# yizuo417/RollingDepth

Hardware: AMD Instinct MI355X
Metric: depth frames/sec at 768px snip_len=3, 1-step denoise; 1/2/4/8 MI355X (higher is better)
Workload: dtype f16; 1 GPU; fast preset: 100-frame 768x768 video, dilations [1, 25] (cap_dilation=True), snippet_len 3, 1-step DDIM, aligner 2000 it, refine 0; SD2-shaped UNet+VAE random-init; preset=fast, frames=100, res=768, parallelism=snippet-dp1

## Files before the change

### include/rdmi.h

```cpp
#ifndef RDMI_H
#define RDMI_H

#include <stddef.h>

#ifdef __cplusplus
extern "C" {
#endif

#define RDMI_OK 0
#define RDMI_E_ARG 1001
#define RDMI_E_ALIGN 1002
#define RDMI_E_UNSUPPORTED 1003

#define RDMI_F16 0
#define RDMI_F32 1
#define RDMI_U8 2
#define RDMI_F32_X3 3
#define RDMI_F32_X6 4

#define RDMI_RESIZE_NEAREST 0
#define RDMI_RESIZE_BILINEAR 1
#define RDMI_RESIZE_BICUBIC 2

#define RDMI_EPI_NONE 0
#define RDMI_EPI_GEGLU 1
#define RDMI_EPI_SILU 2

const char* rdmi_last_error(void);
int rdmi_version(void);

typedef struct rdmi_gemm_args {
  const void* A; long lda; long strideA;
  const void* W; long ldw; long strideW;
  void* C; long ldc; long strideC; int c_f32;
  const float* bias;
  const void* residual; long ldr; long strideR;
  const float* rowbias; int rows_per_group; long rowbias_ld;
  float alpha;
  int M, N, K, batch;
  int epilogue;
  float* gn_part; long gn_ld;
  int dtype;
} rdmi_gemm_args;
int rdmi_gemm(const rdmi_gemm_args* args, void* stream);

typedef struct rdmi_conv_args {
  const void* x; const void* w; void* y;
  const float* bias; const void* residual; const float* rowbias;
  int B, H, W, Cin, Cout, kh, kw, stride, pad_top, pad_left, upsample, Ho, Wo, Kp;
  long y_ld; long res_ld; float alpha; long rowbias_ld;
  float* gn_part; long gn_ld;
  const float* in_mean_rstd; const float* in_gamma; const float* in_beta; int in_groups, in_silu;
  int dtype;
  const void* w_up2;
  const float* in_affine;
} rdmi_conv_args;
int rdmi_conv2d(const rdmi_conv_args* args, void* stream);
int rdmi_conv2d_in_gn_supported(const rdmi_conv_args* args);

long rdmi_groupnorm_workspace(int B, int G);
int rdmi_groupnorm_stats(const void* x, int dtype, int B, long HW, int C, int G, float eps,
                         float* mean_rstd, float* workspace, void* stream);
int rdmi_groupnorm_stats_partials(const float* part, long part_ld, int B, long HW, int C, int G, float eps,
                                  float* mean_rstd, void* stream);
int rdmi_groupnorm_affine(const float* mean_rstd, const float* gamma, const float* beta, int B, int C, int G,
                          float* out, void* stream);
int rdmi_groupnorm_apply(const void* x, void* y, int dtype, int B, long HW, int C, int G,
                         const float* mean_rstd, const float* gamma, const float* beta, int silu,
                         void* stream);

long rdmi_conv3x3_to1_gn_workspace(int B, int H, int W);
int rdmi_conv3x3_to1_gn(const void* x, int dtype, int B, int H, int W, int C, int G, const float* mean_rstd,
                        const float* gamma, const float* beta, int silu, const float* w, float bias,
                        void* y, int y_dtype, float* workspace, void* stream);

int rdmi_layernorm(const void* x, void* y, int dtype, long M, int C, const float* gamma, const float* beta,
                   float eps, void* stream);

int rdmi_attention_fwd(const void* q, const void* k, const void* v, void* o, int B, int H, int Sq,
                       int Sk, int D, long q_ld, long k_ld, long v_ld, long o_ld, long q_bs,
                       long k_bs, long v_bs, long o_bs, float scale, int dtype, void* stream);

int rdmi_attention_smallkv(const void* q, const void* k, const void* v, void* o, int B, int H,
                           int Sq, int L, int D, long q_ld, long o_ld, long q_bs, long o_bs,
                           long kv_bs, float scale, int dtype, void* stream);

int rdmi_cross_attn_pair(const void* x, void* y, long M, int C, int H, const float* ln_gamma,
                         const float* ln_beta, float eps, const float* w, const float* u, const float* c,
                         void* stream);

int rdmi_softmax_rows(const float* s, void* p, long rows, long cols, long p_ld, float scale, int p_dtype,
                      void* stream);

int rdmi_nchw_to_nhwc(const void* x, int x_f32, void* y, int y_dtype, int B, int C, int H, int W, int Cpad,
                      float scale, long x_bstride, long x_cstride, void* stream);
int rdmi_nhwc_to_nchw_f32(const void* x, int dtype, long ld, float* y, int B, int C, int H, int W,
                          float scale, float shift, void* stream);
int rdmi_concat_channels(const void* a, int Ca, const void* b, int Cb, void* y, long P, int dtype, void* stream);
int rdmi_resize_nearest(const void* x, int B, int H, int W, int C, void* y, int Ho, int Wo, int dtype,
                        void* stream);
int rdmi_transpose(const void* src, void* dst, int batch, long rows, long cols, long src_ld,
                   long dst_ld, int dtype, void* stream);
int rdmi_gather_unet_input(const void* rgb, long rgb_frame_ld, const void* depth,
                           long depth_frame_ld, int depth_bcast, const int* frame_idx, int count,
                           long HW, void* out, int dtype, void* stream);
int rdmi_ddim_combine(const void* x, long ld_x, const void* e, long ld_e, void* y, long ld_y,
                      long P, int C, int Cpad, float ca, float cb, float out_scale, long e_period,
                      int dtype, void* stream);
int rdmi_snippet_average(const void* src, int n, int w, int stride, int N, long P, int C, int ld,
                         void* out, int dtype, void* stream);
int rdmi_colorize(const void* depth, int dtype, long n, const void* minmax, const unsigned char* lut, int lut_n,
                  unsigned char* rgb, int* index, void* stream);
int rdmi_snippet_accumulate(const void* src, int dtype, int k0, int nloc, int w, int stride, int N, long P, int C,
                            int ld, double* sum, void* stream);
int rdmi_snippet_finish(const double* sum, int n, int w, int stride, int N, long P, int C, int ld, void* out,
                        int dtype, void* stream);
int rdmi_snippet_average_strided(const void* src, int n, int w, int stride, int start_step, int N, long P, int C,
                                 int ld, void* out, int dtype, void* stream);
int rdmi_snippet_accumulate_strided(const void* src, int dtype, int k0, int nloc, int w, int stride, int start_step,
                                    int N, long P, int C, int ld, double* sum, void* stream);
int rdmi_snippet_finish_strided(const double* sum, int n, int w, int stride, int start_step, int N, long P, int C,
                                int ld, void* out, int dtype, void* stream);
int rdmi_minmax(const void* x, int x_f32, long n, float* minmax, float* workspace, void* stream);
int rdmi_renormalize_f32(float* x, long n, const float* minmax, void* stream);

typedef struct rdmi_aligner_args {
  int n_dil;
  const float* x[8];
  float* s[8]; float* t[8];
  int n[8]; int stride[8];
  int w[8];
  int seq_len; long P;
  float lr, beta1, beta2, eps, lmda2, lmda3, depth_w, loss_scale;
  int iters;
  float* history;
  float* workspace;
  int start_step[8];
} rdmi_aligner_args;
long rdmi_aligner_workspace(const rdmi_aligner_args* a);
int rdmi_aligner_optimize(const rdmi_aligner_args* a, void* stream);
int rdmi_aligner_prepare(const void* x, int x_f32, int n, int w, int H, int W, int border,
                         int factor, const float* shift, float* out, void* stream);
int rdmi_aligner_merge(int n_dil, const void* const* xf, int x_f32, const float* const* s,
                       const float* const* t, const int* n, const int* stride, const int* w, int seq_len,
                       long HW, const float* shift, float* out, void* stream);
int rdmi_aligner_merge_strided(int n_dil, const void* const* xf, int x_f32, const float* const* s,
                               const float* const* t, const int* n, const int* stride, const int* start_step,
                               const int* w, int seq_len, long HW, const float* shift, float* out, void* stream);

int rdmi_aligner_merge_partial_window(int n_dil, const void* const* xf, int x_f32, const float* const* s,
                                      const float* const* t, const int* n, const int* stride, const int* k0,
                                      const int* nloc, const int* w, int f0, int nf, long HW, const float* shift,
                                      double* sum_out, void* stream);
int rdmi_aligner_merge_finish_pieces(int n_dil, const int* n, const int* stride, const int* w, int f0, int nf, long HW,
                                     int npieces, const int* piece_f0, const int* piece_nf, const double* recv,
                                     float* out, void* stream);
int rdmi_aligner_merge_partial_window_strided(int n_dil, const void* const* xf, int x_f32, const float* const* s,
                                              const float* const* t, const int* n, const int* stride,
                                              const int* start_step, const int* k0, const int* nloc, const int* w,
                                              int seq_len, int f0, int nf, long HW, const float* shift,
                                              double* sum_out, void* stream);
int rdmi_aligner_merge_finish_pieces_strided(int n_dil, const int* n, const int* stride, const int* start_step,
                                             const int* w, int seq_len, int f0, int nf, long HW, int npieces,
                                             const int* piece_f0, const int* piece_nf, const double* recv,
                                             float* out, void* stream);

int rdmi_attention_d512(const void* q, const void* k, const void* vt, void* o, int B, int Sq, int Sk, int Skp,
                        long q_ld, long k_ld, long vt_ld, long o_ld, long q_bs, long k_bs, long vt_bs, long o_bs,
                        float scale, int* flags, void* stream);

size_t rdmi_resize_workspace(int N, int C, int H, int W, int Ho, int Wo);
// ... 8 lines not shown
```

### rollingdepth_amd/_native.py

```python
from __future__ import annotations

import ctypes as C
import os

_LIB_PATH = os.environ.get("RDMI_LIB") or os.path.join(os.path.dirname(os.path.abspath(__file__)), "_lib", "librdmi.so")

vp = C.c_void_p
i32 = C.c_int
i64 = C.c_long
f32 = C.c_float


class GemmArgs(C.Structure):
    _fields_ = [
        ("A", vp), ("lda", i64), ("strideA", i64),
        ("W", vp), ("ldw", i64), ("strideW", i64),
        ("C", vp), ("ldc", i64), ("strideC", i64), ("c_f32", i32),
        ("bias", vp),
        ("residual", vp), ("ldr", i64), ("strideR", i64),
        ("rowbias", vp), ("rows_per_group", i32), ("rowbias_ld", i64),
        ("alpha", f32),
        ("M", i32), ("N", i32), ("K", i32), ("batch", i32),
        ("epilogue", i32),
        ("gn_part", vp), ("gn_ld", i64),
        ("dtype", i32),
    ]


class ConvArgs(C.Structure):
    _fields_ = [
        ("x", vp), ("w", vp), ("y", vp),
        ("bias", vp), ("residual", vp), ("rowbias", vp),
        ("B", i32), ("H", i32), ("W", i32), ("Cin", i32), ("Cout", i32), ("kh", i32), ("kw", i32),
        ("stride", i32), ("pad_top", i32), ("pad_left", i32), ("upsample", i32), ("Ho", i32), ("Wo", i32),
        ("Kp", i32),
        ("y_ld", i64), ("res_ld", i64), ("alpha", f32), ("rowbias_ld", i64),
        ("gn_part", vp), ("gn_ld", i64),
        ("in_mean_rstd", vp), ("in_gamma", vp), ("in_beta", vp), ("in_groups", i32), ("in_silu", i32),
        ("dtype", i32),
        ("w_up2", vp),
        ("in_affine", vp),
    ]


class AlignerArgs(C.Structure):
    _fields_ = [
        ("n_dil", i32),
        ("x", vp * 8), ("s", vp * 8), ("t", vp * 8),
        ("n", i32 * 8), ("stride", i32 * 8),
        ("w", i32 * 8), ("seq_len", i32), ("P", i64),
        ("lr", f32), ("beta1", f32), ("beta2", f32), ("eps", f32), ("lmda2", f32), ("lmda3", f32),
        ("depth_w", f32), ("loss_scale", f32),
        ("iters", i32),
        ("history", vp), ("workspace", vp),
        ("start_step", i32 * 8),
    ]


_SIGS = {
    "rdmi_last_error": (C.c_char_p, []),
    "rdmi_version": (i32, []),
    "rdmi_gemm": (i32, [C.POINTER(GemmArgs), vp]),
    "rdmi_conv2d": (i32, [C.POINTER(ConvArgs), vp]),
    "rdmi_conv2d_in_gn_supported": (i32, [C.POINTER(ConvArgs)]),
    "rdmi_groupnorm_workspace": (i64, [i32, i32]),
    "rdmi_groupnorm_stats": (i32, [vp, i32, i32, i64, i32, i32, f32, vp, vp, vp]),
    "rdmi_groupnorm_stats_partials": (i32, [vp, i64, i32, i64, i32, i32, f32, vp, vp]),
    "rdmi_groupnorm_apply": (i32, [vp, vp, i32, i32, i64, i32, i32, vp, vp, vp, i32, vp]),
    "rdmi_conv3x3_to1_gn_workspace": (i64, [i32, i32, i32]),
    "rdmi_conv3x3_to1_gn": (i32, [vp, i32, i32, i32, i32, i32, i32, vp, vp, vp, i32, vp, f32, vp, i32, vp, vp]),
    "rdmi_layernorm": (i32, [vp, vp, i32, i64, i32, vp, vp, f32, vp]),
    "rdmi_attention_fwd": (i32, [vp, vp, vp, vp, i32, i32, i32, i32, i32, i64, i64, i64, i64, i64, i64, i64, i64,
                                 f32, i32, vp]),
    "rdmi_attention_smallkv": (i32, [vp, vp, vp, vp, i32, i32, i32, i32, i32, i64, i64, i64, i64, i64, f32, i32, vp]),
    "rdmi_cross_attn_pair": (i32, [vp, vp, i64, i32, i32, vp, vp, f32, vp, vp, vp, vp]),
    "rdmi_softmax_rows": (i32, [vp, vp, i64, i64, i64, f32, i32, vp]),
    "rdmi_nchw_to_nhwc": (i32, [vp, i32, vp, i32, i32, i32, i32, i32, i32, f32, i64, i64, vp]),
    "rdmi_nhwc_to_nchw_f32": (i32, [vp, i32, i64, vp, i32, i32, i32, i32, f32, f32, vp]),
    "rdmi_concat_channels": (i32, [vp, i32, vp, i32, vp, i64, i32, vp]),
    "rdmi_resize_nearest": (i32, [vp, i32, i32, i32, i32, vp, i32, i32, i32, vp]),
    "rdmi_transpose": (i32, [vp, vp, i32, i64, i64, i64, i64, i32, vp]),
    "rdmi_gather_unet_input": (i32, [vp, i64, vp, i64, i32, vp, i32, i64, vp, i32, vp]),
    "rdmi_ddim_combine": (i32, [vp, i64, vp, i64, vp, i64, i64, i32, i32, f32, f32, f32, i64, i32, vp]),
    "rdmi_snippet_average": (i32, [vp, i32, i32, i32, i32, i64, i32, i32, vp, i32, vp]),
    "rdmi_snippet_accumulate": (i32, [vp, i32, i32, i32, i32, i32, i32, i64, i32, i32, vp, vp]),
    "rdmi_snippet_finish": (i32, [vp, i32, i32, i32, i32, i64, i32, i32, vp, i32, vp]),
    "rdmi_snippet_average_strided": (i32, [vp, i32, i32, i32, i32, i32, i64, i32, i32, vp, i32, vp]),
    "rdmi_snippet_accumulate_strided": (i32, [vp, i32, i32, i32, i32, i32, i32, i32, i64, i32, i32, vp, vp]),
    "rdmi_snippet_finish_strided": (i32, [vp, i32, i32, i32, i32, i32, i64, i32, i32, vp, i32, vp]),
    "rdmi_colorize": (i32, [vp, i32, i64, vp, vp, i32, vp, vp, vp]),
    "rdmi_resize_workspace": (C.c_size_t, [i32, i32, i32, i32, i32, i32]),
    "rdmi_attention_d512": (i32, [vp, vp, vp, vp, i32, i32, i32, i32] + [i64] * 8 + [C.c_float, vp, vp]),
    "rdmi_resize": (i32, [vp, i32, i64, i64, i64, i64, i32, i32, i32, i32, i32, i32, i32, i32, vp, vp, vp]),
    "rdmi_minmax": (i32, [vp, i32, i64, vp, vp, vp]),
    "rdmi_renormalize_f32": (i32, [vp, i64, vp, vp]),
    "rdmi_aligner_workspace": (i64, [C.POINTER(AlignerArgs)]),
    "rdmi_aligner_optimize": (i32, [C.POINTER(AlignerArgs), vp]),
    "rdmi_aligner_prepare": (i32, [vp, i32, i32, i32, i32, i32, i32, i32, vp, vp, vp]),
    "rdmi_aligner_merge": (i32, [i32, C.POINTER(vp), i32, C.POINTER(vp), C.POINTER(vp), C.POINTER(i32),
                                 C.POINTER(i32), C.POINTER(i32), i32, i64, vp, vp, vp]),
    "rdmi_aligner_merge_strided": (i32, [i32, C.POINTER(vp), i32, C.POINTER(vp), C.POINTER(vp), C.POINTER(i32),
                                         C.POINTER(i32), C.POINTER(i32), C.POINTER(i32), i32, i64, vp, vp, vp]),
    "rdmi_groupnorm_affine": (i32, [vp, vp, vp, i32, i32, i32, vp, vp]),
    "rdmi_aligner_merge_partial_window": (i32, [i32, C.POINTER(vp), i32, C.POINTER(vp), C.POINTER(vp),
                                                C.POINTER(i32), C.POINTER(i32), C.POINTER(i32), C.POINTER(i32),
                                                C.POINTER(i32), i32, i32, i64, vp, vp, vp]),
    "rdmi_aligner_merge_finish_pieces": (i32, [i32, C.POINTER(i32), C.POINTER(i32), C.POINTER(i32), i32, i32, i64,
                                               i32, C.POINTER(i32), C.POINTER(i32), vp, vp, vp]),
    "rdmi_aligner_merge_partial_window_strided": (i32, [i32, C.POINTER(vp), i32, C.POINTER(vp), C.POINTER(vp),
                                                        C.POINTER(i32), C.POINTER(i32), C.POINTER(i32),
                                                        C.POINTER(i32), C.POINTER(i32), C.POINTER(i32), i32, i32, i32,
                                                        i64, vp, vp, vp]),
    "rdmi_aligner_merge_finish_pieces_strided": (i32, [i32, C.POINTER(i32), C.POINTER(i32), C.POINTER(i32),
                                                       C.POINTER(i32), i32, i32, i32, i64, i32, C.POINTER(i32),
                                                       C.POINTER(i32), vp, vp, vp]),
}

RDMI_F16, RDMI_F32, RDMI_U8, RDMI_F32_X3, RDMI_F32_X6 = 0, 1, 2, 3, 4
RDMI_RESIZE_NEAREST, RDMI_RESIZE_BILINEAR, RDMI_RESIZE_BICUBIC = 0, 1, 2

EXPORTED = tuple(_SIGS)


def _load():
    if not os.path.exists(_LIB_PATH):
        raise ImportError(
            f"librdmi.so not found at {_LIB_PATH}: build it with `python -m rollingdepth_amd._build` "
            "(the HIP path has no fallback)")
    lib = C.CDLL(_LIB_PATH)
    for name, (res, args) in _SIGS.items():
        fn = getattr(lib, name)
        fn.restype = res
        fn.argtypes = args
    return lib


lib = _load()


class RdmiError(RuntimeError):
    pass


def check(rc: int, what: str = ""):
    if rc != 0:
        msg = lib.rdmi_last_error().decode(errors="replace")
        raise RdmiError(f"{what or 'librdmi'} failed (code {rc}): {msg}")
```

### rollingdepth_amd/csrc/attention.hip

```cpp
#include <stdlib.h>

#include <type_traits>

#include "common.h"

namespace {

struct AttnP {
  const f16* q; const f16* k; const f16* v; f16* o;
  int H, Sq, Sk;
  long q_ld, k_ld, v_ld, o_ld, q_bs, k_bs, v_bs, o_bs;
  float sl2;
  unsigned long long* stamps;
  int sprio;
};

__device__ __forceinline__ unsigned long long attn_stamp() {
  unsigned long long t;
  __builtin_amdgcn_sched_barrier(0);
  asm volatile("s_memtime %0\n\ts_waitcnt lgkmcnt(0)" : "=s"(t) :: "memory");
  __builtin_amdgcn_sched_barrier(0);
  return t;
}

// ... 776 lines not shown
    if constexpr (HC > 0) wave_sum_n<1>(qr, b2); else qr[0] = wave_sum(q);
    const float rstd = rsqrtf(qr[0] / C + eps);
    float n[NV][8], o[NV][8];
#pragma unroll
    for (int i = 0; i < NV; ++i)
#pragma unroll
      for (int e = 0; e < 8; ++e) {
        n[i][e] = lane + 64 * i < CV ? (float)(f16)(((float)v[i][e] - mean) * rstd * gr[i][e] + br[i][e]) : 0.f;
        o[i][e] = 0.f;
      }
    if constexpr (HC > 0) {
      float d[HC];
#pragma unroll
      for (int h = 0; h < HC; ++h) {
        d[h] = 0.f;
#pragma unroll
        for (int i = 0; i < NV; ++i) {
          const int cv = lane + 64 * i;
          if (cv < CV) {
            const f32x4 w0 = *(const f32x4*)(ws + h * C + cv * 8), w1 = *(const f32x4*)(ws + h * C + cv * 8 + 4);
#pragma unroll
            for (int e = 0; e < 4; ++e) d[h] = fmaf(n[i][e], w0[e], fmaf(n[i][4 + e], w1[e], d[h]));
          }
        }
      }
      wave_sum_n<HC>(d, b2);
#pragma unroll
      for (int h = 0; h < HC; ++h) {
        const float ph = 1.0f / (1.0f + __expf(-d[h]));
#pragma unroll
        for (int i = 0; i < NV; ++i) {
          const int cv = lane + 64 * i;
          if (cv < CV) {
            const f32x4 u0 = *(const f32x4*)(us + h * C + cv * 8), u1 = *(const f32x4*)(us + h * C + cv * 8 + 4);
#pragma unroll
            for (int e = 0; e < 4; ++e) {
              o[i][e] = fmaf(ph, u0[e], o[i][e]);
              o[i][4 + e] = fmaf(ph, u1[e], o[i][4 + e]);
            }
          }
        }
      }
    }
    for (int h = 0; h < (HC > 0 ? 0 : H); ++h) {
      float d = 0.f;
#pragma unroll
      for (int i = 0; i < NV; ++i) {
        const int cv = lane + 64 * i;
        if (cv < CV) {
          const f32x4 w0 = *(const f32x4*)(ws + h * C + cv * 8), w1 = *(const f32x4*)(ws + h * C + cv * 8 + 4);
#pragma unroll
          for (int e = 0; e < 4; ++e) d = fmaf(n[i][e], w0[e], fmaf(n[i][4 + e], w1[e], d));
        }
      }
      d = wave_sum(d);
      const float ph = 1.0f / (1.0f + __expf(-d));
#pragma unroll
      for (int i = 0; i < NV; ++i) {
        const int cv = lane + 64 * i;
        if (cv < CV) {
          const f32x4 u0 = *(const f32x4*)(us + h * C + cv * 8), u1 = *(const f32x4*)(us + h * C + cv * 8 + 4);
#pragma unroll
          for (int e = 0; e < 4; ++e) {
            o[i][e] = fmaf(ph, u0[e], o[i][e]);
            o[i][4 + e] = fmaf(ph, u1[e], o[i][4 + e]);
          }
        }
      }
    }
    f16* yr = y + row * C;
#pragma unroll
    for (int i = 0; i < NV; ++i) {
      const int cv = lane + 64 * i;
      if (cv < CV) {
        f16x8 r;
#pragma unroll
        for (int e = 0; e < 8; ++e) r[e] = (f16)((float)v[i][e] + (cr[i][e] + o[i][e]));
        *(f16x8*)(yr + cv * 8) = r;
      }
    }
  }
}

}

extern "C" int rdmi_attention_fwd(const void* q, const void* k, const void* v, void* o, int B, int H, int Sq, int Sk,
                                  int D, long q_ld, long k_ld, long v_ld, long o_ld, long q_bs, long k_bs, long v_bs,
                                  long o_bs, float scale, int dtype, void* stream) {
  RDMI_REQUIRE(q && k && v && o, RDMI_E_ARG, "attention_fwd: null pointer");
  RDMI_REQUIRE(D == 64, RDMI_E_UNSUPPORTED, "attention_fwd: head_dim %d unsupported (64 only)", D);
  RDMI_REQUIRE(B > 0 && H > 0 && Sq > 0 && Sk > 0, RDMI_E_ARG, "attention_fwd: bad sizes");
  if (dtype == RDMI_F32 || dtype == RDMI_F32_X3 || dtype == RDMI_F32_X6)
    return rdmi::attention_fwd_f32(q, k, v, o, B, H, Sq, Sk, q_ld, k_ld, v_ld, o_ld, q_bs, k_bs, v_bs, o_bs, scale,
                                   dtype == RDMI_F32_X3 ? 2 : dtype == RDMI_F32_X6 ? 3 : 1, stream);
  RDMI_REQUIRE(q_ld % 8 == 0 && k_ld % 8 == 0 && v_ld % 8 == 0 && o_ld % 4 == 0 && (((uintptr_t)q | (uintptr_t)k | (uintptr_t)v) & 15) == 0,
               RDMI_E_ALIGN, "attention_fwd: strides/pointers must be 16-byte aligned");
  AttnP p{(const f16*)q, (const f16*)k, (const f16*)v, (f16*)o, H, Sq, Sk, q_ld, k_ld, v_ld, o_ld, q_bs, k_bs, v_bs, o_bs,
          scale * 1.4426950408889634f, nullptr};
  const char* sp = getenv("RDMI_ATTN_SPRIO");
  p.sprio = sp && sp[0] == '1';
  dim3 g(rdmi::div_up(Sq, QB), H, B);
  static const bool f32sum = [] { const char* e = getenv("RDMI_ATTN_F32SUM"); return e && e[0] == '1'; }();
  const char* pe = getenv("RDMI_ATTN_PIPE");
  if (pe && pe[0] == '1' && !f32sum) {
    hipLaunchKernelGGL((attn_fwd_d64_pipe<0, true>), dim3(rdmi::div_up(Sq, pp::QB), H, B), dim3(64 * pp::NW), 0,
                       (hipStream_t)stream, p);
    return rdmi::check_launch("attention_fwd");
  }
  if (!f32sum)
    hipLaunchKernelGGL(attn_fwd_d64<true>, g, dim3(64 * NWV), 0, (hipStream_t)stream, p);
  else
    hipLaunchKernelGGL(attn_fwd_d64<false>, g, dim3(64 * NWV), 0, (hipStream_t)stream, p);
  return rdmi::check_launch("attention_fwd");
}

extern "C" int rdmi_attention_smallkv(const void* q, const void* k, const void* v, void* o, int B, int H, int Sq, int L,
                                      int D, long q_ld, long o_ld, long q_bs, long o_bs, long kv_bs, float scale,
                                      int dtype, void* stream) {
  RDMI_REQUIRE(q && k && v && o, RDMI_E_ARG, "attention_smallkv: null pointer");
  RDMI_REQUIRE(D == 64 && L >= 1 && L <= 16, RDMI_E_UNSUPPORTED, "attention_smallkv: D=%d L=%d unsupported", D, L);
  const size_t esz = dtype == RDMI_F32 ? 4 : 2;
  size_t lds = (size_t)2 * L * H * 64 * esz;
  RDMI_REQUIRE(lds <= 64 * 1024, RDMI_E_UNSUPPORTED, "attention_smallkv: K/V too large for LDS");
  dim3 g(rdmi::div_up((long)Sq * H, 256), B);
  if (dtype == RDMI_F32)
    hipLaunchKernelGGL(attn_smallkv<float>, g, dim3(256), lds, (hipStream_t)stream, (const float*)q, (const float*)k,
                       (const float*)v, (float*)o, H, Sq, L, q_ld, o_ld, q_bs, o_bs, kv_bs, scale);
  else
    hipLaunchKernelGGL(attn_smallkv<f16>, g, dim3(256), lds, (hipStream_t)stream, (const f16*)q, (const f16*)k,
                       (const f16*)v, (f16*)o, H, Sq, L, q_ld, o_ld, q_bs, o_bs, kv_bs, scale);
  return rdmi::check_launch("attention_smallkv");
}

extern "C" int rdmi_softmax_rows(const float* s, void* p, long rows, long cols, long p_ld, float scale, int p_dtype,
                                 void* stream) {
  RDMI_REQUIRE(s && p && rows > 0 && cols > 0 && p_ld >= cols, RDMI_E_ARG, "softmax_rows: bad args");
  hipStream_t st = (hipStream_t)stream;
  if (p_dtype == RDMI_F32) {
    hipLaunchKernelGGL(softmax_rows_k<float>, dim3((unsigned)rows), dim3(256), 0, st, s, (float*)p, cols, p_ld, scale);
    return rdmi::check_launch("softmax_rows");
  }
  const bool vec = cols % 4 == 0 && p_ld % 4 == 0 && ((uintptr_t)s & 15) == 0 && ((uintptr_t)p & 7) == 0;
  const long nv = (cols / 4 + 255) / 256;
  if (vec && nv <= 4)
    hipLaunchKernelGGL(softmax_rows_reg_k<4>, dim3((unsigned)rows), dim3(256), 0, st, s, (f16*)p, cols, p_ld, scale);
  else if (vec && nv <= 16)
    hipLaunchKernelGGL(softmax_rows_reg_k<16>, dim3((unsigned)rows), dim3(256), 0, st, s, (f16*)p, cols, p_ld, scale);
  else
    hipLaunchKernelGGL(softmax_rows_k<f16>, dim3((unsigned)rows), dim3(256), 0, st, s, (f16*)p, cols, p_ld, scale);
  return rdmi::check_launch("softmax_rows");
}

extern "C" int rdmi_cross_attn_pair(const void* x, void* y, long M, int C, int H, const float* ln_gamma,
                                    const float* ln_beta, float eps, const float* w, const float* u, const float* c,
                                    void* stream) {
  RDMI_REQUIRE(x && y && ln_gamma && ln_beta && w && u && c && M > 0 && H > 0, RDMI_E_ARG, "cross_attn_pair: bad args");
  RDMI_REQUIRE(C % 8 == 0 && C <= 64 * 8 * 3, RDMI_E_UNSUPPORTED, "cross_attn_pair: C=%d unsupported", C);
  RDMI_REQUIRE((((uintptr_t)x | (uintptr_t)y | (uintptr_t)w | (uintptr_t)u) & 15) == 0, RDMI_E_ALIGN,
               "cross_attn_pair: pointers must be 16-byte aligned");
  const size_t lds = (size_t)2 * H * C * sizeof(float);
  RDMI_REQUIRE(lds <= 64 * 1024 && H <= 16, RDMI_E_UNSUPPORTED, "cross_attn_pair: H=%d, H*C=%d unsupported", H, H * C);
  long blocks = (M + 3) / 4;
  if (blocks > 4096) blocks = 4096;
  const int nv = (C / 8 + 63) / 64;
#define RDMI_PAIR(NVV, HCC) \
  hipLaunchKernelGGL((attn2_pair_k<NVV, HCC>), dim3((unsigned)blocks), dim3(256), lds, (hipStream_t)stream, \
                     (const f16*)x, (f16*)y, M, C, H, ln_gamma, ln_beta, eps, w, u, c)
  const char* ehc = getenv("RDMI_PAIR_HC");
  const bool hc = !(ehc && ehc[0] == '0');
  if (nv == 1 && H == 5 && hc)
    RDMI_PAIR(1, 5);
  else if (nv == 2 && H == 10 && hc)
    RDMI_PAIR(2, 10);
  else if (nv == 1)
    RDMI_PAIR(1, 0);
  else if (nv == 2)
    RDMI_PAIR(2, 0);
  else
    RDMI_PAIR(3, 0);
#undef RDMI_PAIR
  return rdmi::check_launch("cross_attn_pair");
}
```

### rollingdepth_amd/kernels.py

```python
from __future__ import annotations

import ctypes as C
import math
import os
from typing import Optional, Sequence, Tuple

import torch

from . import _native as _N
from ._native import check, lib

F16 = torch.float16
F32 = torch.float32


def _stream() -> int:
    return torch.cuda.current_stream().cuda_stream


_PROF = None


def profile_start():
    global _PROF
# ... 496 lines not shown
        raise TypeError("groupnorm: out dtype must match x")
    check(lib.rdmi_groupnorm_apply(x.data_ptr(), out.data_ptr(), _dtype_code(x), B, HW, C, groups, mr.data_ptr(),
                                   gamma.data_ptr(), beta.data_ptr(), int(silu), _stream()), "rdmi_groupnorm_apply")
    return out


def conv3x3_to1_gn(x: torch.Tensor, gamma: torch.Tensor, beta: torch.Tensor, groups: int, eps: float, silu: bool,
                   w9: torch.Tensor, bias: float, out: Optional[torch.Tensor] = None,
                   out_dtype: Optional[torch.dtype] = None) -> torch.Tensor:
    _need_act(x, "conv3x3_to1_gn.x")
    _need(w9, F32, "conv3x3_to1_gn.w9")
    B, H, W, C_ = x.shape
    if w9.shape != (9, C_):
        raise ValueError(f"conv3x3_to1_gn: w9 {tuple(w9.shape)} != (9, {C_})")
    mr = groupnorm_stats(x, groups, eps)
    od = out_dtype if out_dtype is not None else (out.dtype if out is not None else x.dtype)
    if od not in (F16, F32):
        raise ValueError(f"conv3x3_to1_gn: output dtype {od} (f16 or f32)")
    out = torch.empty((B, H, W, 1), dtype=od, device=x.device) if out is None else out
    if out.numel() != B * H * W or not out.is_contiguous() or out.dtype != od:
        raise ValueError("conv3x3_to1_gn: out must be a contiguous [B, H, W, 1] tensor of the output dtype")
    ws = _workspace(lib.rdmi_conv3x3_to1_gn_workspace(B, H, W), x.device)
    with _Timed("conv_head", 2.0 * 9 * C_ * B * H * W, f"head B={B} {H}x{W} {C_}->1",
                x.element_size() * B * H * W * C_ + out.element_size() * B * H * W):
        check(lib.rdmi_conv3x3_to1_gn(x.data_ptr(), _dtype_code(x), B, H, W, C_, groups, mr.data_ptr(), gamma.data_ptr(),
                                      beta.data_ptr(), int(silu), w9.data_ptr(), float(bias), out.data_ptr(),
                                      _dtype_code(out), ws.data_ptr(), _stream()), "rdmi_conv3x3_to1_gn")
    return out


def layernorm(x: torch.Tensor, gamma: torch.Tensor, beta: torch.Tensor, eps: float = 1e-5,
              out: Optional[torch.Tensor] = None) -> torch.Tensor:
    _need_act(x, "layernorm.x")
    C_ = x.shape[-1]
    M = x.numel() // C_
    out = torch.empty_like(x) if out is None else out
    check(lib.rdmi_layernorm(x.data_ptr(), out.data_ptr(), _dtype_code(x), M, C_, gamma.data_ptr(), beta.data_ptr(), eps,
                             _stream()), "rdmi_layernorm")
    return out


def attention(q: torch.Tensor, k: torch.Tensor, v: torch.Tensor, heads: int, out: Optional[torch.Tensor] = None,
              scale: Optional[float] = None) -> torch.Tensor:
    _need_act(q, "attention.q")
    for t, nm in ((q, "q"), (k, "k"), (v, "v")):
        _need(t, q.dtype, f"attention.{nm}")
        if t.stride(-1) != 1:
            raise ValueError("attention: inner dim must be contiguous")
    B, Sq, HD = q.shape
    D = HD // heads
    Sk = k.shape[1]
    if out is None:
        out = torch.empty((B, Sq, HD), dtype=q.dtype, device=q.device)
    sc = 1.0 / math.sqrt(D) if scale is None else scale
    code = _dtype_code(q)
    if code == _N.RDMI_F32 and f32_x3("linear"):
        code = _N.RDMI_F32_X3
    elif code == _N.RDMI_F32 and f32_x6():
        code = _N.RDMI_F32_X6
    name = {_N.RDMI_F16: "attention_fwd", _N.RDMI_F32: "attention_fwd_f32", _N.RDMI_F32_X3: "attention_fwd_f32x3",
            _N.RDMI_F32_X6: "attention_fwd_f32x6"}[code]
    es = q.element_size()
    with _Timed(name, 4.0 * B * heads * Sq * Sk * D, f"attn B={B} H={heads} S={Sq}",
                es * B * heads * D * (2 * Sq + 2 * Sk)):
        check(lib.rdmi_attention_fwd(q.data_ptr(), k.data_ptr(), v.data_ptr(), out.data_ptr(), B, heads, Sq, Sk, D,
                                     q.stride(1), k.stride(1), v.stride(1), out.stride(1), q.stride(0), k.stride(0),
                                     v.stride(0), out.stride(0), sc, code, _stream()), "rdmi_attention_fwd")
    return out


def fold_attn2_pair(wq: torch.Tensor, wo: torch.Tensor, bo: torch.Tensor, k2: torch.Tensor, v2: torch.Tensor,
                    heads: int):
    C_ = wq.shape[1]
    d = C_ // heads
    k, v = k2.float(), v2.float()
    dk, dv = (k[1] - k[0]).view(heads, d, 1), (v[1] - v[0]).view(1, heads, d)
    w = (dk * wq.view(heads, d, C_)).sum(1) / math.sqrt(d)
    u = (dv * wo.view(-1, heads, d)).sum(2).t()
    c = wo @ v[0] + bo
    return w.contiguous(), u.contiguous(), c.contiguous()


def cross_attn_pair(x: torch.Tensor, ln_g: torch.Tensor, ln_b: torch.Tensor, eps: float, w: torch.Tensor,
                    u: torch.Tensor, c: torch.Tensor, out: Optional[torch.Tensor] = None) -> torch.Tensor:
    _need(x, F16, "cross_attn_pair.x")
    M, C_ = x.shape
    H = w.shape[0]
    if out is None:
        out = torch.empty_like(x)
    check(lib.rdmi_cross_attn_pair(x.data_ptr(), out.data_ptr(), M, C_, H, ln_g.data_ptr(), ln_b.data_ptr(), eps,
                                   w.data_ptr(), u.data_ptr(), c.data_ptr(), _stream()), "rdmi_cross_attn_pair")
    return out


def attention_smallkv(q: torch.Tensor, k: torch.Tensor, v: torch.Tensor, heads: int,
                      out: Optional[torch.Tensor] = None) -> torch.Tensor:
    _need_act(q, "attention_smallkv.q")
    _need(k, q.dtype, "attention_smallkv.k")
    _need(v, q.dtype, "attention_smallkv.v")
    B, Sq, HD = q.shape
    D = HD // heads
    L = k.shape[1]
    k = k.contiguous()
    v = v.contiguous()
    if out is None:
        out = torch.empty((B, Sq, HD), dtype=q.dtype, device=q.device)
    kv_bs = 0 if k.shape[0] == 1 else k.stride(0)
    check(lib.rdmi_attention_smallkv(q.data_ptr(), k.data_ptr(), v.data_ptr(), out.data_ptr(), B, heads, Sq, L, D,
                                     q.stride(1), out.stride(1), q.stride(0), out.stride(0), kv_bs,
                                     1.0 / math.sqrt(D), _dtype_code(q), _stream()), "rdmi_attention_smallkv")
    return out


def softmax_rows(s: torch.Tensor, scale: float, out: Optional[torch.Tensor] = None, dtype=F16) -> torch.Tensor:
    _need(s, F32, "softmax_rows.s")
    cols = s.shape[-1]
    rows = s.numel() // cols
    out = torch.empty(s.shape, dtype=dtype, device=s.device) if out is None else out
    p_ld = out.shape[-1]
    if out.numel() != rows * p_ld or not out.is_contiguous() or p_ld < cols:
        raise ValueError("softmax_rows: out must be a contiguous [..., >= cols] tensor")
    check(lib.rdmi_softmax_rows(s.data_ptr(), out.data_ptr(), rows, cols, p_ld, scale, _dtype_code(out), _stream()),
          "rdmi_softmax_rows")
    return out


def attention_1head(q: torch.Tensor, k: torch.Tensor, v: torch.Tensor, scale: float) -> torch.Tensor:
    B, Sq, D = q.shape
    Sk = k.shape[1]
    if D == 512 and q.dtype == F16 and os.environ.get("RDMI_VAE_FLASH", "1") != "0":
        return attention_d512(q, k, v, scale)
    s = gemm(q, k, D, out_f32=True)
    Sp = (Sk + 7) // 8 * 8
    p = softmax_rows(s, scale, out=torch.empty((B, Sq, Sp), dtype=q.dtype, device=q.device))
    del s
    vt = torch.zeros((B, D, Sp), dtype=q.dtype, device=q.device) if Sp != Sk else None
    vt = transpose(v, out=vt)
    return gemm(p, vt, Sp)


def attention_d512(q: torch.Tensor, k: torch.Tensor, v: torch.Tensor, scale: float) -> torch.Tensor:
    B, Sq, D = q.shape
    Sk = k.shape[1]
    if D != 512 or q.dtype != F16 or k.dtype != F16 or v.dtype != F16:
        raise ValueError("attention_d512: f16 q / k / v with head dim 512")
    Skp = (Sk + 31) // 32 * 32
    vt = torch.zeros((B, D, Skp), dtype=F16, device=q.device) if Skp != Sk else None
    vt = transpose(v, out=vt)
    o = torch.empty((B, Sq, D), dtype=F16, device=q.device)
    flags = None
    if os.environ.get("RDMI_D512_W4", "0") == "1":
        flags = torch.empty((B * ((Sq + 127) // 128),), dtype=torch.int32, device=q.device)
    with _Timed("attention_d512", 4.0 * B * Sq * Sk * D, f"attn512 B={B} S={Sq}", 2 * B * D * (2 * Sq + 2 * Sk)):
        check(lib.rdmi_attention_d512(q.data_ptr(), k.data_ptr(), vt.data_ptr(), o.data_ptr(), B, Sq, Sk, Skp,
                                      q.stride(1), k.stride(1), vt.stride(1), o.stride(1), q.stride(0), k.stride(0),
                                      vt.stride(0), o.stride(0), float(scale),
                                      flags.data_ptr() if flags is not None else None, _stream()),
              "rdmi_attention_d512")
    return o


def transpose(src: torch.Tensor, out: Optional[torch.Tensor] = None) -> torch.Tensor:
    _need_act(src, "transpose.src")
    B, R, Cc = src.shape
    out = torch.empty((B, Cc, R), dtype=src.dtype, device=src.device) if out is None else out
    for t, rows, nm in ((src, R, "src"), (out, Cc, "out")):
        if t.stride(2) != 1 or (B > 1 and t.stride(0) != rows * t.stride(1)):
            raise ValueError(f"transpose: {nm} strides {t.stride()} (unit column stride, batch stride = rows · row "
                             f"stride expected)")
    check(lib.rdmi_transpose(src.data_ptr(), out.data_ptr(), B, R, Cc, src.stride(1), out.stride(1), _dtype_code(src),
                             _stream()), "rdmi_transpose")
    return out


def nchw_to_nhwc(x: torch.Tensor, cpad: int, scale: float = 1.0, dtype=F16) -> torch.Tensor:
# ... 332 lines not shown
```

### rollingdepth_amd/unet.py

```python
from __future__ import annotations

import math
import os
from typing import Dict, Optional

import numpy as np
import torch

from . import kernels as K
from .config import unet_heads, validate_unet_config

F16, F32 = torch.float16, torch.float32


def _sinusoid(t: int, dim: int, flip: bool, shift: float) -> np.ndarray:
    half = dim // 2
    ex = -math.log(10000) * np.arange(half, dtype=np.float32) / (half - shift)
    e = np.float32(t) * np.exp(ex.astype(np.float32)).astype(np.float32)
    e = np.concatenate([np.sin(e), np.cos(e)]).astype(np.float32)
    if flip:
        e = np.concatenate([e[half:], e[:half]])
    return e


# ... 32 lines not shown

class _Norm:
    def __init__(self, sd, key, dev):
        self.g = sd[key + ".weight"].to(dev, F32)
        self.b = sd[key + ".bias"].to(dev, F32)


class Resnet:

    def __init__(self, sd, p, dev, groups, eps, temb_slot=None, dtype=F16):
        self.n1 = _Norm(sd, p + ".norm1", dev)
        self.c1 = _Conv(sd, p + ".conv1", dev, dtype=dtype)
        self.n2 = _Norm(sd, p + ".norm2", dev)
        self.c2 = _Conv(sd, p + ".conv2", dev, dtype=dtype)
        self.sc = _Conv(sd, p + ".conv_shortcut", dev, pad=0, dtype=dtype) if p + ".conv_shortcut.weight" in sd \
            else None
        self.groups, self.eps = groups, eps
        self.temb_slot = temb_slot

    def __call__(self, x, temb_all=None):
        rb = None
        if self.temb_slot is not None and temb_all is not None:
            o, w = self.temb_slot
            rb = temb_all[o:o + w]
        h = self.c1.normed(x, self.n1, self.groups, self.eps, rowbias=rb, gn=True)
        res = self.sc(x) if self.sc is not None else x
        return self.c2.normed(h, self.n2, self.groups, self.eps, residual=res, gn=True)


class Transformer:

    def __init__(self, sd, p, dev, heads, groups, dtype=F16):
        self.heads, self.groups = heads, groups
        self.norm = _Norm(sd, p + ".norm", dev)
        self.proj_in = _Lin(sd, p + ".proj_in", dev, dtype=dtype)
        self.proj_out = _Lin(sd, p + ".proj_out", dev, dtype=dtype)
        q = p + ".transformer_blocks.0"
        self.ln1 = _Norm(sd, q + ".norm1", dev)
        self.ln2 = _Norm(sd, q + ".norm2", dev)
        self.ln3 = _Norm(sd, q + ".norm3", dev)
        wqkv = torch.cat([sd[f"{q}.attn1.to_{n}.weight"] for n in ("q", "k", "v")], 0)
        self.c = wqkv.shape[1]
        self.qkv = K.pack_linear(wqkv, dev, dtype)
        self.o1 = _Lin(sd, q + ".attn1.to_out.0", dev, dtype=dtype)
        self.q2 = _Lin(sd, q + ".attn2.to_q", dev, bias=False, dtype=dtype)
        self.k2 = _Lin(sd, q + ".attn2.to_k", dev, bias=False, dtype=dtype)
        self.v2 = _Lin(sd, q + ".attn2.to_v", dev, bias=False, dtype=dtype)
        self.o2 = _Lin(sd, q + ".attn2.to_out.0", dev, dtype=dtype)
        wp, bp = K.geglu_permute(sd[q + ".ff.net.0.proj.weight"], sd[q + ".ff.net.0.proj.bias"])
        self.ff1_w = K.pack_linear(wp, dev, dtype)
        self.ff1_b = bp.to(dev, F32)
        self.ff2 = _Lin(sd, q + ".ff.net.2", dev, dtype=dtype)
        self._ctx_key = None
        self._pair = None
        self._pair_w = None
        if dtype == F16 and 2 * heads * self.c * 4 <= 64 * 1024 and heads <= 16 and \
                os.environ.get("RDMI_ATTN2_PAIR", "1") != "0":
            self._pair_w = (sd[q + ".attn2.to_q.weight"].half().float().to(dev),
                            sd[q + ".attn2.to_out.0.weight"].half().float().to(dev),
                            sd.get(q + ".attn2.to_out.0.bias", torch.zeros(self.c)).float().to(dev))

    def set_context(self, ctx16: torch.Tensor):
        if self._ctx_key is ctx16:
            return
        self.k2c = K.gemm(ctx16, self.k2.w, self.k2.k)
        self.v2c = K.gemm(ctx16, self.v2.w, self.v2.k)
        self._ctx_key = ctx16
        self._pair = None
        if self._pair_w is not None and self.k2c.shape[0] == 1 and self.k2c.shape[1] == 2:
            self._pair = K.fold_attn2_pair(*self._pair_w, self.k2c[0], self.v2c[0], self.heads)

    def __call__(self, x, num_view: Optional[int]):
        B, H, W, C = x.shape
        HW = H * W
        t = K.groupnorm(x, self.norm.g, self.norm.b, self.groups, 1e-6, silu=False)
        t = self.proj_in(t.view(B * HW, C))
        n1 = K.layernorm(t, self.ln1.g, self.ln1.b, 1e-5)
        qkv = K.gemm(n1, self.qkv, C)
        nv = num_view or 1
        bb = B // nv
        qkv3 = qkv.view(bb, nv * HW, 3 * C)
        o = K.attention(qkv3[..., :C], qkv3[..., C:2 * C], qkv3[..., 2 * C:], self.heads)
        t = self.o1(o.view(B * HW, C), residual=t)
        if self._pair is not None:
            t = K.cross_attn_pair(t, self.ln2.g, self.ln2.b, 1e-5, *self._pair)
        else:
            n2 = K.layernorm(t, self.ln2.g, self.ln2.b, 1e-5)
            q2 = self.q2(n2)
            kv_b = self.k2c.shape[0]
            if kv_b == 1:
                o2 = K.attention_smallkv(q2.view(1, B * HW, C), self.k2c, self.v2c, self.heads)
            else:
                o2 = K.attention_smallkv(q2.view(kv_b, -1, C), self.k2c, self.v2c, self.heads)
            t = self.o2(o2.view(B * HW, C), residual=t)
        n3 = K.layernorm(t, self.ln3.g, self.ln3.b, 1e-5)
        f = K.gemm(n3, self.ff1_w, C, bias=self.ff1_b, geglu=True)
        t = self.ff2(f, residual=t)
        out = self.proj_out(t, residual=x.view(B * HW, C), gn=True)
        return K.gn_view(out, (B, H, W, C))


class UNet:

    def __init__(self, cfg: dict, sd: Dict[str, torch.Tensor], device, dtype=F16):
        dev = torch.device(device)
        if dtype not in (F16, F32):
            raise NotImplementedError(f"UNet storage dtype {dtype} (f16 or f32)")
        validate_unet_config(cfg)
        self.cfg, self.dev, self.dtype = cfg, dev, dtype
        g, eps = cfg["norm_num_groups"], cfg["norm_eps"]
        heads = unet_heads(cfg)
        ch = cfg["block_out_channels"]
        L = cfg["layers_per_block"]
        self.ch, self.L = ch, L
        self.in_ch = cfg["in_channels"]
        self.out_ch = cfg["out_channels"]
        self.conv_in = _Conv(sd, "conv_in", dev, dtype=dtype)
        self.t1 = _Lin(sd, "time_embedding.linear_1", dev, dtype=dtype)
        self.t2 = _Lin(sd, "time_embedding.linear_2", dev, dtype=dtype)
        tp_w, tp_b, off = [], [], 0
        slots = {}
        for k in sd:
            if k.endswith("time_emb_proj.weight"):
                p = k[: -len(".time_emb_proj.weight")]
                w = sd[k]
                tp_w.append(w)
                tp_b.append(sd[p + ".time_emb_proj.bias"])
                slots[p] = (off, w.shape[0])
                off += w.shape[0]
        self.tp_w = K.pack_linear(torch.cat(tp_w, 0), dev, dtype)
        self.tp_b = torch.cat(tp_b, 0).to(dev, F32)
        self.tp_k = tp_w[0].shape[1]
        self._temb_cache = {}

        def R(p):
            return Resnet(sd, p, dev, g, eps, slots.get(p), dtype=dtype)

        self.down = []
        for i, bt in enumerate(cfg["down_block_types"]):
            blk = {"res": [], "attn": [], "ds": None}
            for j in range(L):
                blk["res"].append(R(f"down_blocks.{i}.resnets.{j}"))
                if bt == "CrossAttnDownBlock2D":
                    blk["attn"].append(Transformer(sd, f"down_blocks.{i}.attentions.{j}", dev, heads[i], g, dtype))
            if i < len(ch) - 1:
                blk["ds"] = _Conv(sd, f"down_blocks.{i}.downsamplers.0.conv", dev, stride=2, pad=1, dtype=dtype)
            self.down.append(blk)
        self.mid_res = [R("mid_block.resnets.0"), R("mid_block.resnets.1")]
        self.mid_attn = Transformer(sd, "mid_block.attentions.0", dev, heads[-1], g, dtype)
        rheads = list(reversed(heads))
        self.up = []
        for i, bt in enumerate(cfg["up_block_types"]):
            blk = {"res": [], "attn": [], "us": None}
            for j in range(L + 1):
                blk["res"].append(R(f"up_blocks.{i}.resnets.{j}"))
                if bt == "CrossAttnUpBlock2D":
                    blk["attn"].append(Transformer(sd, f"up_blocks.{i}.attentions.{j}", dev, rheads[i], g, dtype))
            if i < len(ch) - 1:
                blk["us"] = _Conv(sd, f"up_blocks.{i}.upsamplers.0.conv", dev, dtype=dtype, up2=True)
            self.up.append(blk)
        self.norm_out = _Norm(sd, "conv_norm_out", dev)
        self.conv_out = _Conv(sd, "conv_out", dev, dtype=dtype)
        self.groups, self.eps = g, eps
        self.transformers = [t for b in self.down for t in b["attn"]] + [self.mid_attn] + \
                            [t for b in self.up for t in b["attn"]]

    def time_embedding(self, t: int) -> torch.Tensor:
        e = self._temb_cache.get(int(t))
        if e is not None:
            return e
        s = _sinusoid(int(t), self.ch[0], self.cfg.get("flip_sin_to_cos", True), self.cfg.get("freq_shift", 0))
        x = torch.from_numpy(s).to(self.dev, self.dtype).view(1, -1)
        h = K.gemm(x, self.t1.w, self.t1.k, bias=self.t1.b, silu=True)
        emb = K.gemm(h, self.t2.w, self.t2.k, bias=self.t2.b, silu=True)
        proj = K.gemm(emb, self.tp_w, self.tp_k, bias=self.tp_b, out_f32=True)
        e = proj.view(-1)
        self._temb_cache[int(t)] = e
        return e
# ... 37 lines not shown
```

Measured before the change: 23.96 depth frames/s.

## Fuse LayerNorm3 into cross-attention pair kernel with persistent prefetching blocks

Adds a new cross-attention pair kernel that fuses the following LayerNorm (ln3) into the same pass, so the residual output is normalized while it is still in registers instead of being re-read by a separate layernorm launch. The kernel uses a persistent grid sized to the number of resident blocks, a 3-deep row prefetch ring, and hand-written DPP/permlane wave reductions for the per-head dot products. The UNet transformer block uses the fused output for ln3 when the folded pair path is active. The change adds inline assembly specific to the target ISA and an extra output buffer, and keeps an env-controlled fallback.

```diff
diff --git a/include/rdmi.h b/include/rdmi.h
--- a/include/rdmi.h
+++ b/include/rdmi.h
@@ -87,6 +87,7 @@
 
 int rdmi_cross_attn_pair(const void* x, void* y, long M, int C, int H, const float* ln_gamma,
                          const float* ln_beta, float eps, const float* w, const float* u, const float* c,
+                         void* y3, const float* ln3_gamma, const float* ln3_beta, float eps3, int impl,
                          void* stream);
 
 int rdmi_softmax_rows(const float* s, void* p, long rows, long cols, long p_ld, float scale, int p_dtype,
diff --git a/rollingdepth_amd/_native.py b/rollingdepth_amd/_native.py
--- a/rollingdepth_amd/_native.py
+++ b/rollingdepth_amd/_native.py
@@ -73,7 +73,7 @@
     "rdmi_attention_fwd": (i32, [vp, vp, vp, vp, i32, i32, i32, i32, i32, i64, i64, i64, i64, i64, i64, i64, i64,
                                  f32, i32, vp]),
     "rdmi_attention_smallkv": (i32, [vp, vp, vp, vp, i32, i32, i32, i32, i32, i64, i64, i64, i64, i64, f32, i32, vp]),
-    "rdmi_cross_attn_pair": (i32, [vp, vp, i64, i32, i32, vp, vp, f32, vp, vp, vp, vp]),
+    "rdmi_cross_attn_pair": (i32, [vp, vp, i64, i32, i32, vp, vp, f32, vp, vp, vp, vp, vp, vp, f32, i32, vp]),
     "rdmi_softmax_rows": (i32, [vp, vp, i64, i64, i64, f32, i32, vp]),
     "rdmi_nchw_to_nhwc": (i32, [vp, i32, vp, i32, i32, i32, i32, i32, i32, f32, i64, i64, vp]),
     "rdmi_nhwc_to_nchw_f32": (i32, [vp, i32, i64, vp, i32, i32, i32, i32, f32, f32, vp]),
diff --git a/rollingdepth_amd/csrc/attention.hip b/rollingdepth_amd/csrc/attention.hip
--- a/rollingdepth_amd/csrc/attention.hip
+++ b/rollingdepth_amd/csrc/attention.hip
@@ -882,6 +882,231 @@
   }
 }
 
+__device__ __forceinline__ float swap32_pair(float a, float b) {
+  asm("s_nop 1\n\tv_permlane32_swap_b32 %0, %1\n\ts_nop 1" : "+v"(a), "+v"(b));
+  return a + b;
+}
+__device__ __forceinline__ float swap_quad(float a, float b, float c, float d) {
+  asm("s_nop 1\n\t"
+      "v_permlane32_swap_b32 %0, %1\n\t"
+      "v_permlane32_swap_b32 %2, %3\n\t"
+      "s_nop 1\n\t"
+      "v_add_f32 %0, %0, %1\n\t"
+      "v_add_f32 %2, %2, %3\n\t"
+      "s_nop 1\n\t"
+      "v_permlane16_swap_b32 %0, %2\n\t"
+      "s_nop 1\n\t"
+      "v_add_f32 %0, %0, %2"
+      : "+v"(a), "+v"(b), "+v"(c), "+v"(d));
+  return a;
+}
+__device__ __forceinline__ float row_sum(float d) {
+  float t;
+  asm("s_nop 1\n\t"
+      "v_add_f32_dpp %0, %0, %0 row_ror:8 row_mask:0xf bank_mask:0xf\n\t"
+      "s_nop 1\n\t"
+      "v_add_f32_dpp %1, %0, %0 row_ror:12 row_mask:0xf bank_mask:0x5\n\t"
+      "v_add_f32_dpp %1, %0, %0 row_ror:4 row_mask:0xf bank_mask:0xa\n\t"
+      "s_nop 1\n\t"
+      "v_add_f32_dpp %1, %1, %1 quad_perm:[2,3,0,1] row_mask:0xf bank_mask:0xf\n\t"
+      "s_nop 1\n\t"
+      "v_add_f32_dpp %1, %1, %1 quad_perm:[1,0,3,2] row_mask:0xf bank_mask:0xf"
+      : "+v"(d), "=&v"(t));
+  return t;
+}
+__device__ __forceinline__ float wave_sum_1(float v) {
+  return row_sum(swap_sum<false>(swap_sum<true>(v)));
+}
+constexpr int pair_head_lane(int HC, int h) {
+  const int g = h / 4, k = h % 4, n = HC - 4 * g < 4 ? HC - 4 * g : 4;
+  const int row = n >= 3 ? (k == 0 ? 0 : k == 1 ? 2 : k == 2 ? 1 : 3) : n == 2 ? 2 * k : 0;
+  return 16 * row + g;
+}
+template <int HC, int G = 0>
+__device__ __forceinline__ float pair_head_sums(const float (&d)[HC], int lane, float m = 0.f) {
+  static_assert(HC <= 64, "one lane column per group of four heads");
+  constexpr int n = HC - 4 * G < 4 ? HC - 4 * G : 4;
+  float q;
+  if constexpr (n == 4)
+    q = swap_quad(d[4 * G], d[4 * G + 1], d[4 * G + 2], d[4 * G + 3]);
+  else if constexpr (n == 3)
+    q = swap_quad(d[4 * G], d[4 * G + 1], d[4 * G + 2], 0.f);
+  else if constexpr (n == 2)
+    q = swap_sum<false>(swap32_pair(d[4 * G], d[4 * G + 1]));
+  else
+    q = swap_sum<false>(swap_sum<true>(d[4 * G]));
+  q = row_sum(q);
+  m = G == 0 || (lane & 15) == G ? q : m;
+  if constexpr (4 * (G + 1) < HC)
+    return pair_head_sums<HC, G + 1>(d, lane, m);
+  else
+    return m;
+}
+__device__ __forceinline__ float sq_acc(float q, float d) {
+#pragma clang fp contract(off)
+  const float p = d * d;
+  return q + p;
+}
+
+template <int NV, int HC, bool LN3>
+__global__ __launch_bounds__(256) __attribute__((amdgpu_waves_per_eu(NV == 1 ? 4 : 2))) void attn2_pair_pk_k(const f16* __restrict__ x, f16* __restrict__ y,
+                                                       f16* __restrict__ y3, long M, int C,
+                                                       const float* __restrict__ g, const float* __restrict__ b,
+                                                       float eps, const float* __restrict__ wd,
+                                                       const float* __restrict__ u, const float* __restrict__ c0,
+                                                       const float* __restrict__ g3, const float* __restrict__ b3,
+                                                       float eps3) {
+  extern __shared__ __attribute__((aligned(16))) float sm[];
+  for (int i = threadIdx.x; i < HC * C / 4; i += 256) {
+    ((f32x4*)sm)[i] = ((const f32x4*)wd)[i];
+    ((f32x4*)sm)[HC * C / 4 + i] = ((const f32x4*)u)[i];
+  }
+  __syncthreads();
+  const float* ws = sm;
+  const float* us = sm + HC * C;
+  const int lane = threadIdx.x & 63;
+  const int CV = C >> 3;
+  float gr[NV][8], br[NV][8], cr[NV][8], g3r[LN3 ? NV : 1][8], b3r[LN3 ? NV : 1][8];
+#pragma unroll
+  for (int i = 0; i < NV; ++i) {
+    const int cv = lane + 64 * i;
+#pragma unroll
+    for (int e = 0; e < 8; ++e) {
+      const int cc = cv < CV ? cv * 8 + e : 0;
+      gr[i][e] = g[cc];
+      br[i][e] = b[cc];
+      cr[i][e] = c0[cc];
+      if constexpr (LN3) {
+        g3r[i][e] = g3[cc];
+        b3r[i][e] = b3[cc];
+      }
+    }
+  }
+  constexpr int PF = 3;
+  const long stride = gridDim.x * 4L;
+  long row = blockIdx.x * 4L + (threadIdx.x >> 6);
+  f16x8 ring[PF][NV];
+  auto load = [&](long r, f16x8 (&dst)[NV]) {
+#pragma unroll
+    for (int i = 0; i < NV; ++i) {
+      const int cv = lane + 64 * i;
+      if (r < M && cv < CV) dst[i] = *(const f16x8*)(x + r * C + cv * 8);
+    }
+  };
+#pragma unroll
+  for (int p = 0; p < PF; ++p) load(row + p * stride, ring[p]);
+  while (row < M) {
+#pragma unroll
+    for (int p = 0; p < PF; ++p) {
+      if (row >= M) break;
+      float xf[NV][8];
+#pragma unroll
+      for (int i = 0; i < NV; ++i)
+#pragma unroll
+        for (int e = 0; e < 8; ++e) xf[i][e] = (float)ring[p][i][e];
+      load(row + PF * stride, ring[p]);
+      float st[1] = {0.f};
+#pragma unroll
+      for (int i = 0; i < NV; ++i)
+        if (lane + 64 * i < CV)
+#pragma unroll
+          for (int e = 0; e < 8; ++e) st[0] += xf[i][e];
+      st[0] = wave_sum_1(st[0]);
+      const float mean = st[0] / C;
+      float qt[1] = {0.f};
+#pragma unroll
+      for (int i = 0; i < NV; ++i)
+        if (lane + 64 * i < CV)
+#pragma unroll
+          for (int e = 0; e < 8; ++e) qt[0] = sq_acc(qt[0], xf[i][e] - mean);
+      qt[0] = wave_sum_1(qt[0]);
+      const float rstd = rsqrtf(qt[0] / C + eps);
+      float d[HC];
+#pragma unroll
+      for (int h = 0; h < HC; ++h) d[h] = 0.f;
+#pragma unroll
+      for (int i = 0; i < NV; ++i) {
+        const int cv = lane + 64 * i;
+        if (cv < CV) {
+          float n[8];
+#pragma unroll
+          for (int e = 0; e < 8; ++e) n[e] = (float)(f16)fmaf((xf[i][e] - mean) * rstd, gr[i][e], br[i][e]);
+#pragma unroll
+          for (int h = 0; h < HC; ++h) {
+            const f32x4 w0 = *(const f32x4*)(ws + h * C + cv * 8), w1 = *(const f32x4*)(ws + h * C + cv * 8 + 4);
+#pragma unroll
+            for (int e = 0; e < 4; ++e) d[h] = fmaf(n[e], w0[e], fmaf(n[4 + e], w1[e], d[h]));
+          }
+        }
+      }
+      const float sig = 1.0f / (1.0f + __expf(-pair_head_sums<HC>(d, lane)));
+      float ph[HC];
+#pragma unroll
+      for (int h = 0; h < HC; ++h)
+        ph[h] = __builtin_bit_cast(float, __builtin_amdgcn_readlane(__builtin_bit_cast(int, sig), pair_head_lane(HC, h)));
+      float rf[NV][8];
+#pragma unroll
+      for (int i = 0; i < NV; ++i) {
+        const int cv = lane + 64 * i;
+        if (cv < CV) {
+          float o[8];
+#pragma unroll
+          for (int e = 0; e < 8; ++e) o[e] = 0.f;
+#pragma unroll
+          for (int h = 0; h < HC; ++h) {
+            const f32x4 u0 = *(const f32x4*)(us + h * C + cv * 8), u1 = *(const f32x4*)(us + h * C + cv * 8 + 4);
+#pragma unroll
+            for (int e = 0; e < 4; ++e) {
+              o[e] = fmaf(ph[h], u0[e], o[e]);
+              o[4 + e] = fmaf(ph[h], u1[e], o[4 + e]);
+            }
+          }
+          f16x8 r;
+#pragma unroll
+          for (int e = 0; e < 8; ++e) {
+            r[e] = (f16)(xf[i][e] + (cr[i][e] + o[e]));
+            rf[i][e] = (float)r[e];
+          }
+          *(f16x8*)(y + row * C + cv * 8) = r;
+        }
+      }
+      if constexpr (LN3) {
+        float s3[1] = {0.f};
+#pragma unroll
+        for (int i = 0; i < NV; ++i)
+          if (lane + 64 * i < CV)
+#pragma unroll
+            for (int e = 0; e < 8; ++e) s3[0] += rf[i][e];
+        s3[0] = wave_sum_1(s3[0]);
+        const float mean3 = s3[0] / C;
+        float q3[1] = {0.f};
+#pragma unroll
+        for (int i = 0; i < NV; ++i)
+          if (lane + 64 * i < CV)
+#pragma unroll
+            for (int e = 0; e < 8; ++e) q3[0] = sq_acc(q3[0], rf[i][e] - mean3);
+        q3[0] = wave_sum_1(q3[0]);
+        const float rstd3 = rsqrtf(q3[0] / C + eps3);
+#pragma unroll
+        for (int i = 0; i < NV; ++i) {
+          const int cv = lane + 64 * i;
+          if (cv < CV) {
+            f16x8 r;
+#pragma unroll
+            for (int e = 0; e < 8; ++e) {
+              float t = fmaf((rf[i][e] - mean3) * rstd3, g3r[i][e], b3r[i][e]);
+              asm("" : "+v"(t));
+              r[e] = (f16)t;
+            }
+            *(f16x8*)(y3 + row * C + cv * 8) = r;
+          }
+        }
+      }
+      row += stride;
+    }
+  }
+}
+
 }
 
 extern "C" int rdmi_attention_fwd(const void* q, const void* k, const void* v, void* o, int B, int H, int Sq, int Sk,
@@ -951,23 +1176,60 @@
   return rdmi::check_launch("softmax_rows");
 }
 
+namespace {
+template <typename K>
+long resident_blocks(K k, size_t lds) {
+  int per_cu = 0, dev = 0, cus = 0;
+  if (hipOccupancyMaxActiveBlocksPerMultiprocessor(&per_cu, k, 256, lds) != hipSuccess || per_cu < 1) per_cu = 1;
+  if (hipGetDevice(&dev) != hipSuccess ||
+      hipDeviceGetAttribute(&cus, hipDeviceAttributeMultiprocessorCount, dev) != hipSuccess || cus < 1)
+    cus = 256;
+  return (long)per_cu * cus;
+}
+}
+
 extern "C" int rdmi_cross_attn_pair(const void* x, void* y, long M, int C, int H, const float* ln_gamma,
                                     const float* ln_beta, float eps, const float* w, const float* u, const float* c,
+                                    void* y3, const float* ln3_gamma, const float* ln3_beta, float eps3, int impl,
                                     void* stream) {
   RDMI_REQUIRE(x && y && ln_gamma && ln_beta && w && u && c && M > 0 && H > 0, RDMI_E_ARG, "cross_attn_pair: bad args");
   RDMI_REQUIRE(C % 8 == 0 && C <= 64 * 8 * 3, RDMI_E_UNSUPPORTED, "cross_attn_pair: C=%d unsupported", C);
-  RDMI_REQUIRE((((uintptr_t)x | (uintptr_t)y | (uintptr_t)w | (uintptr_t)u) & 15) == 0, RDMI_E_ALIGN,
+  RDMI_REQUIRE((((uintptr_t)x | (uintptr_t)y | (uintptr_t)y3 | (uintptr_t)w | (uintptr_t)u) & 15) == 0, RDMI_E_ALIGN,
                "cross_attn_pair: pointers must be 16-byte aligned");
+  RDMI_REQUIRE(!y3 || (ln3_gamma && ln3_beta && y3 != y && y3 != x), RDMI_E_ARG, "cross_attn_pair: bad LN3 args");
   const size_t lds = (size_t)2 * H * C * sizeof(float);
   RDMI_REQUIRE(lds <= 64 * 1024 && H <= 16, RDMI_E_UNSUPPORTED, "cross_attn_pair: H=%d, H*C=%d unsupported", H, H * C);
   long blocks = (M + 3) / 4;
+  const int nv = (C / 8 + 63) / 64;
+  static const bool pack_env = [] { const char* e = getenv("RDMI_PAIR_PACK"); return !(e && e[0] == '0'); }();
+  const char* ehc = getenv("RDMI_PAIR_HC");
+  const bool hc = !(ehc && ehc[0] == '0');
+  if ((impl < 0 ? pack_env : impl != 0) && hc && ((nv == 1 && H == 5) || (nv == 2 && H == 10))) {
+#define RDMI_PAIR_PK(NVV, HCC, L3)                                                                              \
+  do {                                                                                                          \
+    static thread_local size_t res_lds = 0;                                                                     \
+    static thread_local long res = 0;                                                                           \
+    if (res_lds != lds) res = resident_blocks(attn2_pair_pk_k<NVV, HCC, L3>, lds), res_lds = lds;               \
+    if (blocks > res) blocks = res;                                                                             \
+    hipLaunchKernelGGL((attn2_pair_pk_k<NVV, HCC, L3>), dim3((unsigned)blocks), dim3(256), lds,                 \
+                       (hipStream_t)stream, (const f16*)x, (f16*)y, (f16*)y3, M, C, ln_gamma, ln_beta, eps, w, u, \
+                       c, ln3_gamma, ln3_beta, eps3);                                                           \
+  } while (0)
+    if (nv == 1 && y3)
+      RDMI_PAIR_PK(1, 5, true);
+    else if (nv == 1)
+      RDMI_PAIR_PK(1, 5, false);
+    else if (y3)
+      RDMI_PAIR_PK(2, 10, true);
+    else
+      RDMI_PAIR_PK(2, 10, false);
+#undef RDMI_PAIR_PK
+    return rdmi::check_launch("cross_attn_pair");
+  }
   if (blocks > 4096) blocks = 4096;
-  const int nv = (C / 8 + 63) / 64;
 #define RDMI_PAIR(NVV, HCC) \
   hipLaunchKernelGGL((attn2_pair_k<NVV, HCC>), dim3((unsigned)blocks), dim3(256), lds, (hipStream_t)stream, \
                      (const f16*)x, (f16*)y, M, C, H, ln_gamma, ln_beta, eps, w, u, c)
-  const char* ehc = getenv("RDMI_PAIR_HC");
-  const bool hc = !(ehc && ehc[0] == '0');
   if (nv == 1 && H == 5 && hc)
     RDMI_PAIR(1, 5);
   else if (nv == 2 && H == 10 && hc)
@@ -979,5 +1241,7 @@
   else
     RDMI_PAIR(3, 0);
 #undef RDMI_PAIR
-  return rdmi::check_launch("cross_attn_pair");
-}
+  const int rc = rdmi::check_launch("cross_attn_pair");
+  if (rc || !y3) return rc;
+  return rdmi_layernorm(y, y3, RDMI_F16, M, C, ln3_gamma, ln3_beta, eps3, stream);
+}
diff --git a/rollingdepth_amd/kernels.py b/rollingdepth_amd/kernels.py
--- a/rollingdepth_amd/kernels.py
+++ b/rollingdepth_amd/kernels.py
@@ -602,15 +602,21 @@
 
 
 def cross_attn_pair(x: torch.Tensor, ln_g: torch.Tensor, ln_b: torch.Tensor, eps: float, w: torch.Tensor,
-                    u: torch.Tensor, c: torch.Tensor, out: Optional[torch.Tensor] = None) -> torch.Tensor:
+                    u: torch.Tensor, c: torch.Tensor, out: Optional[torch.Tensor] = None,
+                    ln3: Optional[tuple] = None, impl: int = -1):
     _need(x, F16, "cross_attn_pair.x")
     M, C_ = x.shape
     H = w.shape[0]
     if out is None:
         out = torch.empty_like(x)
+    out3, a3 = None, (None, None, None, 0.0)
+    if ln3 is not None:
+        out3 = torch.empty_like(out)
+        a3 = (out3.data_ptr(), ln3[0].data_ptr(), ln3[1].data_ptr(), ln3[2])
     check(lib.rdmi_cross_attn_pair(x.data_ptr(), out.data_ptr(), M, C_, H, ln_g.data_ptr(), ln_b.data_ptr(), eps,
-                                   w.data_ptr(), u.data_ptr(), c.data_ptr(), _stream()), "rdmi_cross_attn_pair")
-    return out
+                                   w.data_ptr(), u.data_ptr(), c.data_ptr(), *a3, impl, _stream()),
+          "rdmi_cross_attn_pair")
+    return out if ln3 is None else (out, out3)
 
 
 def attention_smallkv(q: torch.Tensor, k: torch.Tensor, v: torch.Tensor, heads: int,
diff --git a/rollingdepth_amd/unet.py b/rollingdepth_amd/unet.py
--- a/rollingdepth_amd/unet.py
+++ b/rollingdepth_amd/unet.py
@@ -138,8 +138,10 @@
         qkv3 = qkv.view(bb, nv * HW, 3 * C)
         o = K.attention(qkv3[..., :C], qkv3[..., C:2 * C], qkv3[..., 2 * C:], self.heads)
         t = self.o1(o.view(B * HW, C), residual=t)
+        n3 = None
         if self._pair is not None:
-            t = K.cross_attn_pair(t, self.ln2.g, self.ln2.b, 1e-5, *self._pair)
+            t, n3 = K.cross_attn_pair(t, self.ln2.g, self.ln2.b, 1e-5, *self._pair,
+                                      ln3=(self.ln3.g, self.ln3.b, 1e-5))
         else:
             n2 = K.layernorm(t, self.ln2.g, self.ln2.b, 1e-5)
             q2 = self.q2(n2)
@@ -149,7 +151,8 @@
             else:
                 o2 = K.attention_smallkv(q2.view(kv_b, -1, C), self.k2c, self.v2c, self.heads)
             t = self.o2(o2.view(B * HW, C), residual=t)
-        n3 = K.layernorm(t, self.ln3.g, self.ln3.b, 1e-5)
+        if n3 is None:
+            n3 = K.layernorm(t, self.ln3.g, self.ln3.b, 1e-5)
         f = K.gemm(n3, self.ff1_w, C, bias=self.ff1_b, geglu=True)
         t = self.ff2(f, residual=t)
         out = self.proj_out(t, residual=x.view(B * HW, C), gn=True)
```

Measured after the change: 24.01 depth frames/s, median of 6. Within noise of the previous version (+0.2%).
